# opentrack/neuralnet-tracker-traincode

Measured on AMD Instinct MI355X. Metric: face-crops/sec fwd+bwd @ batch 512, higher is better.
Workload: dtype f32; 1 GPU; NetworkWithPointHead(mobilenetv1, point head on, NLL off = training-script defaults): zero_grad + fwd + multi-task loss + bwd + fused clip/Adam step; per_gpu_batch=512, global_batch=512, input=129x129x1 f32, parallelism=dp1

## Files before the change

### neuralnet-tracker-traincode_amd/csrc/pw_bwd_fused.hip

```cpp
#include "ttk_common.h"
#include "conv_geom.h"

namespace ttk {

typedef float f32x16 __attribute__((ext_vector_type(16)));

constexpr int kFusedBM = 64;

template <int CIN, int COUT>
struct FusedShape {
  static constexpr int LDY = COUT + 4, LDC = CIN + 4, LDW = COUT + 4;
  static constexpr int NTC = CIN / 32, MTO = COUT / 32;
  static constexpr int DG = 2 * NTC;
  static constexpr int WG = MTO * NTC;
  static constexpr size_t smem_floats = (size_t)CIN * LDW + 2 * kFusedBM * LDY + 2 * kFusedBM * LDC + 4 * 2 * CIN;
};

template <int CIN, int COUT>
__global__ void __launch_bounds__(512) pw_bwd_fused_k(const float* __restrict__ g, const float* __restrict__ y, const float* __restrict__ bn_pw,
                                                       const float* __restrict__ w, const float* __restrict__ ydw,
                                                       const float* __restrict__ bn_dw, float* __restrict__ g_dw, float* __restrict__ dW,
                                                       float* __restrict__ wpartial, float* __restrict__ part, int64_t M, int ntiles) {
  using S = FusedShape<CIN, COUT>;
  constexpr int BM = kFusedBM, LDY = S::LDY, LDC = S::LDC, LDW = S::LDW, NTC = S::NTC, DG = S::DG, WG = S::WG;
  static_assert((CIN == 32 && COUT == 64) || (CIN == 64 && COUT == 128), "shapes of the first two pointwise layers");
  constexpr int DGW = DG >= 4 ? DG / 4 : 1, WGW = WG >= 4 ? WG / 4 : 1;
  static_assert(DGW == 1, "one data-gradient tile per consumer wave");
  __shared__ __attribute__((aligned(16))) float smem[S::smem_floats];
  float* Wt = smem;
  float* DyS = Wt + CIN * LDW;
  float* YcS = DyS + 2 * BM * LDY;
  float* red = YcS + 2 * BM * LDC;
  const int tid = threadIdx.x, lane = tid & 63, wave = tid >> 6;
  const bool producer = wave >= 4;
  const int r32 = lane & 31, h = lane >> 5;
  constexpr bool WG_PROD = false;
  const int wgw = WG_PROD ? wave - 4 : wave;
  const bool has_wg = WG_PROD ? producer : (!producer && (WG >= 4 || wave >= 4 - WG));
  const int wj0 = WG >= 4 ? wgw * WGW : wgw - (4 - WG);
  f32x16 wacc[WGW];
  float wsc[WGW], wbe[WGW];
#pragma unroll
  for (int j = 0; j < WGW; ++j) {
#pragma unroll
    for (int e = 0; e < 16; ++e) wacc[j][e] = 0.f;
    const int col = ((has_wg ? wj0 + j : 0) % NTC) * 32 + r32;
    wsc[j] = bn_dw[TTK_BN_SCALE * CIN + col];
    wbe[j] = bn_dw[TTK_BN_BETA * CIN + col];
  }
  auto wgrad_jobs = [&](int st, auto&& between) {
    const float* Dy = DyS + st * BM * LDY;
    const float* Yc = YcS + st * BM * LDC;
#pragma unroll
    for (int j = 0; j < WGW; ++j) {
      const int mt = (wj0 + j) / NTC, nt = (wj0 + j) % NTC;
      const float* ap = Dy + (4 * h) * LDY + mt * 32 + r32;
      const float* bp = Yc + (4 * h) * LDC + nt * 32 + r32;
      float a[2][4], b[2][4];
#pragma unroll
      for (int i = 0; i < 4; ++i) { a[0][i] = ap[i * LDY]; b[0][i] = bp[i * LDC]; }
#pragma unroll
      for (int q = 0; q < BM / 8; ++q) {
        const int cur = q & 1;
        if (q + 1 < BM / 8) {
#pragma unroll
          for (int i = 0; i < 4; ++i) { a[cur ^ 1][i] = ap[(8 * (q + 1) + i) * LDY]; b[cur ^ 1][i] = bp[(8 * (q + 1) + i) * LDC]; }
        }
        __builtin_amdgcn_sched_barrier(0);
#pragma unroll
        for (int i = 0; i < 4; ++i)
          wacc[j] = __builtin_amdgcn_mfma_f32_32x32x2f32(a[cur][i], fmaxf(fmaf(wsc[j], b[cur][i], wbe[j]), 0.f), wacc[j], 0, 0, 0);
        between(j * (BM / 8) + q);
        __builtin_amdgcn_sched_barrier(0);
      }
    }
  };

  for (int i = tid; i < CIN * COUT; i += 512) {
    const int co = i / CIN, ci = i - co * CIN;
    Wt[ci * LDW + co] = w[i];
  }

  if (producer) {
    const int pt = tid - 256;
    constexpr int QY = COUT / 4, QC = CIN / 4;
    constexpr int NY = BM * QY / 256, NC = BM * QC / 256;
    const int cy = pt % QY, cc = pt % QC;
    const float4 ga = ld4(bn_pw + TTK_BN_GA * COUT + 4 * cy), gb = ld4(bn_pw + TTK_BN_GB * COUT + 4 * cy);
    const float4 gmean = ld4(bn_pw + TTK_BN_GMEAN * COUT + 4 * cy), ymean = ld4(bn_pw + TTK_BN_MEAN * COUT + 4 * cy);
    const float4 dmean = ld4(bn_dw + TTK_BN_MEAN * CIN + 4 * cc);
    float4 rg[NY], ry[NY], rc[NC];
    auto load = [&](int t) {
      const int64_t m0 = (int64_t)t * BM;
#pragma unroll
      for (int i = 0; i < NY; ++i) {
        const int64_t row = m0 + (pt + 256 * i) / QY;
        const int64_t rcl = row < M ? row : M - 1;
        rg[i] = ld4nt(g + act_off(rcl, 4 * cy, M));
        ry[i] = ld4nt(y + act_off(rcl, 4 * cy, M));
      }
#pragma unroll
      for (int i = 0; i < NC; ++i) {
        const int64_t row = m0 + (pt + 256 * i) / QC;
        const int64_t rcl = row < M ? row : M - 1;
        rc[i] = ld4(ydw + act_off(rcl, 4 * cc, M));
      }
    };
    auto store = [&](int t, int st) {
      const int64_t m0 = (int64_t)t * BM;
#pragma unroll
      for (int i = 0; i < NY; ++i) {
        const int r = (pt + 256 * i) / QY;
        float4 v = fma4(ga, sub4(rg[i], gmean), mul4(gb, sub4(ry[i], ymean)));
        if (m0 + r >= M) v = f4(0.f);
        st4(DyS + (st * BM + r) * LDY + 4 * cy, v);
      }
#pragma unroll
      for (int i = 0; i < NC; ++i) {
        const int r = (pt + 256 * i) / QC;
        st4(YcS + (st * BM + r) * LDC + 4 * cc, sub4(rc[i], dmean));
      }
    };
    int t = blockIdx.x;
    if (t < ntiles) {
      load(t);
      store(t, 0);
      if (t + (int)gridDim.x < ntiles) load(t + gridDim.x);
    }
    __syncthreads();
    for (int it = 0; t < ntiles; t += gridDim.x, ++it) {
      const int tn = t + gridDim.x;
      if (tn < ntiles) {
        store(tn, (it + 1) & 1);
        if (tn + (int)gridDim.x < ntiles) load(tn + gridDim.x);
      }
      if constexpr (WG_PROD) wgrad_jobs(it & 1, [](int) {});
      __syncthreads();
    }
  } else {
    const bool has_dg = DG >= 4 || wave < DG;
    const int dj0 = DG >= 4 ? wave * DGW : wave;
    float s1[DGW], s2[DGW], dsc[DGW], dbe[DGW];
#pragma unroll
    for (int j = 0; j < DGW; ++j) {
      const int col = ((dj0 + j) % NTC) * 32 + r32;
      s1[j] = 0.f; s2[j] = 0.f;
      dsc[j] = has_dg ? bn_dw[TTK_BN_SCALE * CIN + col] : 0.f;
      dbe[j] = has_dg ? bn_dw[TTK_BN_BETA * CIN + col] : 0.f;
    }
    __syncthreads();
    int it = 0;
    for (int t = blockIdx.x; t < ntiles; t += gridDim.x, ++it) {
      const int st = it & 1;
      const float* Dy = DyS + st * BM * LDY;
      const float* Yc = YcS + st * BM * LDC;
      const int64_t m0 = (int64_t)t * BM;
      if (has_dg) {
#pragma unroll
        for (int j = 0; j < DGW; ++j) {
          const int mt = (dj0 + j) / NTC, nt = (dj0 + j) % NTC;
          f32x16 acc;
#pragma unroll
          for (int e = 0; e < 16; ++e) acc[e] = 0.f;
          const float* ap = Dy + (mt * 32 + r32) * LDY + 4 * h;
          const float* bp = Wt + (nt * 32 + r32) * LDW + 4 * h;
          float4 a4[2], b4[2];
          a4[0] = ld4(ap); b4[0] = ld4(bp);
#pragma unroll
          for (int q = 0; q < COUT / 8; ++q) {
            const int cur = q & 1;
            if (q + 1 < COUT / 8) { a4[cur ^ 1] = ld4(ap + 8 * (q + 1)); b4[cur ^ 1] = ld4(bp + 8 * (q + 1)); }
            __builtin_amdgcn_sched_barrier(0);
            acc = __builtin_amdgcn_mfma_f32_32x32x2f32(a4[cur].x, b4[cur].x, acc, 0, 0, 0);
            acc = __builtin_amdgcn_mfma_f32_32x32x2f32(a4[cur].y, b4[cur].y, acc, 0, 0, 0);
            acc = __builtin_amdgcn_mfma_f32_32x32x2f32(a4[cur].z, b4[cur].z, acc, 0, 0, 0);
            acc = __builtin_amdgcn_mfma_f32_32x32x2f32(a4[cur].w, b4[cur].w, acc, 0, 0, 0);
            __builtin_amdgcn_sched_barrier(0);
          }
          const int col = nt * 32 + r32;
          auto epi = [&](int e) {
            const int row = mt * 32 + (e & 3) + 8 * (e >> 2) + 4 * h;
            const float yc = Yc[row * LDC + col];
            const float out = fmaf(dsc[j], yc, dbe[j]) > 0.f ? acc[e] : 0.f;
            if (m0 + row < M) {
              g_dw[act_off(m0 + row, col, M)] = out;
              s1[j] += out;
              s2[j] = fmaf(out, yc, s2[j]);
            }
          };
          if constexpr (!WG_PROD && WG >= 4 && WGW * (BM / 8) == 16) {
            wgrad_jobs(st, epi);
          } else {
#pragma unroll
            for (int e = 0; e < 16; ++e) epi(e);
          }
        }
      }
      if constexpr (!WG_PROD && !(WG >= 4 && WGW * (BM / 8) == 16))
        if (has_wg) wgrad_jobs(st, [](int) {});
      __syncthreads();
    }
#pragma unroll
    for (int j = 0; j < DGW; ++j) {
      s1[j] += __shfl_xor(s1[j], 32);
      s2[j] += __shfl_xor(s2[j], 32);
    }
    if (has_dg && h == 0) {
      static_assert(DGW == 1, "one data-gradient tile per wave");
      red[(wave * 2 + 0) * CIN + (dj0 % NTC) * 32 + r32] = s1[0];
      red[(wave * 2 + 1) * CIN + (dj0 % NTC) * 32 + r32] = s2[0];
    }
  }
  if (has_wg) {
#pragma unroll
    for (int j = 0; j < WGW; ++j) {
      const int mt = (wj0 + j) / NTC, nt = (wj0 + j) % NTC;
#pragma unroll
      for (int e = 0; e < 16; ++e) {
        const int co = mt * 32 + (e & 3) + 8 * (e >> 2) + 4 * h, ci = nt * 32 + r32;
        if (wpartial) wpartial[(size_t)blockIdx.x * COUT * CIN + co * CIN + ci] = wacc[j][e];
        else atomicAdd(dW + co * CIN + ci, wacc[j][e]);
      }
    }
  }
  __syncthreads();
  if (part && tid < 2 * CIN) {
    const int which = tid / CIN, c = tid % CIN, nt = c / 32;
    float a = 0.f;
    for (int wv = 0; wv < (DG >= 4 ? 4 : DG); ++wv)
      if (wv % NTC == nt) a += red[(wv * 2 + which) * CIN + c];
    part[(size_t)blockIdx.x * 2 * CIN + which * CIN + c] = a;
  }
}


typedef _Float16 fz16x8 __attribute__((ext_vector_type(8)));
typedef _Float16 fz16x2 __attribute__((ext_vector_type(2)));
typedef float fz32x2 __attribute__((ext_vector_type(2)));
typedef float fz32x4 __attribute__((ext_vector_type(4)));

__device__ __forceinline__ int fz_swz(int row, int chunk) { return row * 32 + ((chunk ^ ((row >> 3) & 1)) << 4); }
__device__ __forceinline__ void fz_split(fz32x4 v, uint2& h, uint2& l) {
  const fz16x2 h01 = __builtin_convertvector(fz32x2{v.x, v.y}, fz16x2), h23 = __builtin_convertvector(fz32x2{v.z, v.w}, fz16x2);
  const fz32x2 f01 = __builtin_convertvector(h01, fz32x2), f23 = __builtin_convertvector(h23, fz32x2);
  const fz16x2 l01 = __builtin_convertvector(fz32x2{v.x - f01.x, v.y - f01.y}, fz16x2);
  const fz16x2 l23 = __builtin_convertvector(fz32x2{v.z - f23.x, v.w - f23.y}, fz16x2);
  h = make_uint2(__builtin_bit_cast(unsigned, h01), __builtin_bit_cast(unsigned, h23));
  l = make_uint2(__builtin_bit_cast(unsigned, l01), __builtin_bit_cast(unsigned, l23));
}

constexpr int kF16BM = 32;
template <int CIN, int COUT>
struct F16Shape {
  static constexpr int RowPlane = kF16BM * COUT * 2;
  static constexpr int TPlaneY = COUT * 32;
  static constexpr int TPlaneA = CIN * 32;
  static constexpr int Ldc = CIN + 4;
  static constexpr int Stage = 2 * RowPlane + 2 * 2 * TPlaneY + 2 * 2 * TPlaneA + kF16BM * Ldc * 4;
  static constexpr int NCI = CIN / 32, NCO = COUT / 32;
  static constexpr int GROUPS = 4 / NCI;
  static constexpr int COW = NCO / GROUPS;
};

template <int CIN, int COUT>
__global__ void __launch_bounds__(512) __attribute__((amdgpu_waves_per_eu(2, 2)))
pw_bwd_fused16_k(const float* __restrict__ g, const float* __restrict__ y, const float* __restrict__ bn_pw, const uint16_t* __restrict__ wq,
                 const float* __restrict__ wraw, const float* __restrict__ wmax, const float* __restrict__ ydw, const float* __restrict__ bn_dw, float* __restrict__ g_dw,
                 float* __restrict__ dW, float* __restrict__ wpartial, float* __restrict__ part, int64_t M, int ntiles) {
  using S_ = F16Shape<CIN, COUT>;
  constexpr int BM = kF16BM, NCI = S_::NCI, COW = S_::COW, kStage = S_::Stage, kRowPlane = S_::RowPlane, kTY = S_::TPlaneY, kTA = S_::TPlaneA,
                kLdc = S_::Ldc;
  static_assert((CIN == 128 || CIN == 64) && COUT == 128, "shapes");
  __shared__ __attribute__((aligned(16))) unsigned char lds[2 * kStage + 4 * 2 * 32 * 4];
  float* red = reinterpret_cast<float*>(lds + 2 * kStage);
  const int tid = threadIdx.x, lane = tid & 63, wave = tid >> 6;
  const bool producer = wave >= 4;
  const int r32 = lane & 31, h = lane >> 5;
  const float sa = pow2_scale(bn_pw[(size_t)TTK_BN_AUX * COUT + TTK_AUX_DY_BOUND]);
  const float sx = pow2_scale(bn_dw[(size_t)TTK_BN_AUX * CIN + TTK_AUX_ACT_BOUND]);
  const float sw = pow2_scale(*wmax);
  auto stage_ptr = [&](int st) { return lds + st * kStage; };

  if (producer) {
    const int pt = tid - 256;
    const int mb = pt & 7, cq = pt >> 3;
    const bool a_on = cq < CIN / 4;
    const int cqa = a_on ? cq : 0;
    const int sub = mb >> 2, chunk = (mb >> 1) & 1, o8 = (mb & 1) * 8;
    const fz32x4 ga = *reinterpret_cast<const fz32x4*>(bn_pw + TTK_BN_GA * COUT + 4 * cq) * sa;
    const fz32x4 gb = *reinterpret_cast<const fz32x4*>(bn_pw + TTK_BN_GB * COUT + 4 * cq) * sa;
    const fz32x4 gmean = *reinterpret_cast<const fz32x4*>(bn_pw + TTK_BN_GMEAN * COUT + 4 * cq);
    const fz32x4 ymean = *reinterpret_cast<const fz32x4*>(bn_pw + TTK_BN_MEAN * COUT + 4 * cq);
    const fz32x4 dsc = *reinterpret_cast<const fz32x4*>(bn_dw + TTK_BN_SCALE * CIN + 4 * cqa) * sx;
    const fz32x4 dbe = *reinterpret_cast<const fz32x4*>(bn_dw + TTK_BN_BETA * CIN + 4 * cqa) * sx;
    const fz32x4 dmean = *reinterpret_cast<const fz32x4*>(bn_dw + TTK_BN_MEAN * CIN + 4 * cqa);
    fz32x4 rg[4], ry[4], rc[4];
    auto load = [&](int t) {
      const int64_t r0 = (int64_t)t * BM + 4 * mb;
#pragma unroll
      for (int i = 0; i < 4; ++i) {
        const int64_t row = r0 + i < M ? r0 + i : M - 1;
        const float4 a = ld4nt(g + act_off(row, 4 * cq, M)), b = ld4nt(y + act_off(row, 4 * cq, M));
        rg[i] = fz32x4{a.x, a.y, a.z, a.w}; ry[i] = fz32x4{b.x, b.y, b.z, b.w};
        if (a_on) {
          const float4 c = ld4(ydw + act_off(row, 4 * cqa, M));
          rc[i] = fz32x4{c.x, c.y, c.z, c.w};
        }
      }
    };
    auto store = [&](int t, int st) {
      unsigned char* S = stage_ptr(st);
      unsigned char* DyR = S;
      unsigned char* DyT = S + 2 * kRowPlane;
      unsigned char* AT = DyT + 2 * 2 * kTY;
      float* Yc = reinterpret_cast<float*>(AT + 2 * 2 * kTA);
      const int64_t r0 = (int64_t)t * BM + 4 * mb;
      fz32x4 dy[4], av[4];
#pragma unroll
      for (int i = 0; i < 4; ++i) {
        dy[i] = ga * (rg[i] - gmean) + gb * (ry[i] - ymean);
        if (r0 + i >= M) dy[i] = fz32x4{0.f, 0.f, 0.f, 0.f};
        uint2 ph, pl;
        fz_split(dy[i], ph, pl);
        const int row = 4 * mb + i, off = row * (COUT * 2) + ((((cq >> 1) ^ (row & 15))) << 4) + (cq & 1) * 8;
        *reinterpret_cast<uint2*>(DyR + off) = ph;
        *reinterpret_cast<uint2*>(DyR + kRowPlane + off) = pl;
        if (a_on) {
          const fz32x4 yc = rc[i] - dmean;
          fz32x4 a = dsc * yc + dbe;
          a.x = fmaxf(a.x, 0.f); a.y = fmaxf(a.y, 0.f); a.z = fmaxf(a.z, 0.f); a.w = fmaxf(a.w, 0.f);
          if (r0 + i >= M) a = fz32x4{0.f, 0.f, 0.f, 0.f};
          av[i] = a;
          *reinterpret_cast<fz32x4*>(Yc + (4 * mb + i) * kLdc + 4 * cqa) = yc;
        }
      }
#pragma unroll
      for (int e = 0; e < 4; ++e) {
        uint2 ph, pl;
        fz_split(fz32x4{dy[0][e], dy[1][e], dy[2][e], dy[3][e]}, ph, pl);
        const int offy = sub * (2 * kTY) + fz_swz(4 * cq + e, chunk) + o8;
        *reinterpret_cast<uint2*>(DyT + offy) = ph;
        *reinterpret_cast<uint2*>(DyT + kTY + offy) = pl;
        if (a_on) {
          fz_split(fz32x4{av[0][e], av[1][e], av[2][e], av[3][e]}, ph, pl);
          const int offa = sub * (2 * kTA) + fz_swz(4 * cqa + e, chunk) + o8;
          *reinterpret_cast<uint2*>(AT + offa) = ph;
          *reinterpret_cast<uint2*>(AT + kTA + offa) = pl;
        }
      }
    };
    int t = blockIdx.x;
    if (t < ntiles) {
      load(t);
      store(t, 0);
      if (t + (int)gridDim.x < ntiles) load(t + gridDim.x);
    }
    __syncthreads();
    for (int it = 0; t < ntiles; t += gridDim.x, ++it) {
      const int tn = t + gridDim.x;
      if (tn < ntiles) {
        store(tn, (it + 1) & 1);
        if (tn + (int)gridDim.x < ntiles) load(tn + gridDim.x);
      }
      __syncthreads();
    }
  } else {
    const bool has_dg = wave < NCI;
    const int cit = wave % NCI, cog = wave / NCI;
    const int ci_dg = 32 * (has_dg ? wave : 0) + r32, ci_wg = 32 * cit + r32;
    fz16x8 Wf[COUT / 16][2];
#pragma unroll
    for (int s = 0; s < COUT / 16; ++s) {
      const int co = 16 * s + 8 * h;
      if (CIN == 128) {
        const size_t idx = ((size_t)(co >> 5) * CIN + ci_dg) * 32 + (co & 31);
        Wf[s][0] = *reinterpret_cast<const fz16x8*>(wq + idx);
        Wf[s][1] = *reinterpret_cast<const fz16x8*>(wq + (size_t)CIN * COUT + idx);
      } else {
#pragma unroll
        for (int e = 0; e < 8; ++e) {
          const float xs = wraw[(size_t)(co + e) * CIN + ci_dg] * sw;
          const _Float16 hh = (_Float16)xs;
          Wf[s][0][e] = hh;
          Wf[s][1][e] = (_Float16)(xs - (float)hh);
        }
      }
    }
    const float dsc = bn_dw[TTK_BN_SCALE * CIN + ci_dg], dbe = bn_dw[TTK_BN_BETA * CIN + ci_dg];
    const float inv_dg = 1.f / (sa * sw), inv_wg = 1.f / (sa * sx);
    f32x16 wacc[COW];
#pragma unroll
    for (int tt = 0; tt < COW; ++tt)
#pragma unroll
      for (int e = 0; e < 16; ++e) wacc[tt][e] = 0.f;
    float s1 = 0.f, s2 = 0.f;
    __syncthreads();
    int it = 0;
    for (int t = blockIdx.x; t < ntiles; t += gridDim.x, ++it) {
      const unsigned char* S = stage_ptr(it & 1);
      const unsigned char* DyR = S;
      const unsigned char* DyT = S + 2 * kRowPlane;
      const unsigned char* AT = DyT + 2 * 2 * kTY;
      const float* Yc = reinterpret_cast<const float*>(AT + 2 * 2 * kTA);
      const int64_t m0 = (int64_t)t * BM;
      f32x16 acc;
#pragma unroll
      for (int e = 0; e < 16; ++e) acc[e] = 0.f;
      if (has_dg) {
#pragma unroll
        for (int s = 0; s < COUT / 16; ++s) {
          const int off = r32 * (COUT * 2) + ((((2 * s + h) ^ (r32 & 15))) << 4);
          const fz16x8 ah = *reinterpret_cast<const fz16x8*>(DyR + off), al = *reinterpret_cast<const fz16x8*>(DyR + kRowPlane + off);
          acc = __builtin_amdgcn_mfma_f32_32x32x16_f16(ah, Wf[s][1], acc, 0, 0, 0);
          acc = __builtin_amdgcn_mfma_f32_32x32x16_f16(al, Wf[s][0], acc, 0, 0, 0);
          acc = __builtin_amdgcn_mfma_f32_32x32x16_f16(ah, Wf[s][0], acc, 0, 0, 0);
        }
      }
      fz16x8 bh[2], bl[2];
#pragma unroll
      for (int s = 0; s < 2; ++s) {
        const int off = s * (2 * kTA) + fz_swz(ci_wg, h);
        bh[s] = *reinterpret_cast<const fz16x8*>(AT + off);
        bl[s] = *reinterpret_cast<const fz16x8*>(AT + kTA + off);
      }
#pragma unroll
      for (int tt = 0; tt < COW; ++tt)
#pragma unroll
        for (int s = 0; s < 2; ++s) {
          const int off = s * (2 * kTY) + fz_swz(32 * (cog * COW + tt) + r32, h);
          const fz16x8 ah = *reinterpret_cast<const fz16x8*>(DyT + off), al = *reinterpret_cast<const fz16x8*>(DyT + kTY + off);
          wacc[tt] = __builtin_amdgcn_mfma_f32_32x32x16_f16(ah, bl[s], wacc[tt], 0, 0, 0);
          wacc[tt] = __builtin_amdgcn_mfma_f32_32x32x16_f16(al, bh[s], wacc[tt], 0, 0, 0);
          wacc[tt] = __builtin_amdgcn_mfma_f32_32x32x16_f16(ah, bh[s], wacc[tt], 0, 0, 0);
        }
      if (has_dg) {
#pragma unroll
        for (int e = 0; e < 16; ++e) {
          const int row = (e & 3) + 8 * (e >> 2) + 4 * h;
          const float yc = Yc[row * kLdc + ci_dg];
          const float out = fmaf(dsc, yc, dbe) > 0.f ? acc[e] * inv_dg : 0.f;
          if (m0 + row < M) {
            g_dw[act_off(m0 + row, ci_dg, M)] = out;
            s1 += out;
            s2 = fmaf(out, yc, s2);
          }
        }
      }
      __syncthreads();
    }
#pragma unroll
    for (int tt = 0; tt < COW; ++tt)
#pragma unroll
      for (int e = 0; e < 16; ++e) {
        const int co = 32 * (cog * COW + tt) + (e & 3) + 8 * (e >> 2) + 4 * h;
        const float v = wacc[tt][e] * inv_wg;
        if (wpartial) wpartial[(size_t)blockIdx.x * COUT * CIN + co * CIN + ci_wg] = v;
        else atomicAdd(dW + co * CIN + ci_wg, v);
      }
    s1 += __shfl_xor(s1, 32);
    s2 += __shfl_xor(s2, 32);
    if (h == 0 && has_dg) { red[(wave * 2 + 0) * 32 + r32] = s1; red[(wave * 2 + 1) * 32 + r32] = s2; }
  }
  __syncthreads();
  if (part && tid < 2 * CIN) {
    const int which = tid / CIN, c = tid % CIN;
    part[(size_t)blockIdx.x * 2 * CIN + which * CIN + c] = red[((c >> 5) * 2 + which) * 32 + (c & 31)];
  }
}

static bool fused_f16(int Cin) { return Cin == 128 || (Cin == 64 && gemm_mode() == GEMM_F16X2 && !exp_env("TTK_FUSED_FP32")); }
static bool fused_shape(int Cin, int Cout) {
  return (Cin == 32 && Cout == 64) || (Cin == 64 && Cout == 128) || (Cin == 128 && Cout == 128 && gemm_mode() == GEMM_F16X2);
}

static int fused_grid(int64_t M, int Cin) {
  const int64_t ntiles = ceil_div(M, fused_f16(Cin) ? kF16BM : kFusedBM);
  const int64_t cap = Cin == 32 ? 512 : 256;
  return (int)(ntiles < cap ? ntiles : cap);
}

}

using namespace ttk;

extern "C" {

int ttk_pwconv1x1_bwd_fused_rows(int64_t M, int Cin, int Cout) { return fused_shape(Cin, Cout) && M > 0 ? fused_grid(M, Cin) : 0; }

size_t ttk_pwconv1x1_bwd_fused_partial_bytes(int64_t M, int Cin, int Cout) {
  return fused_shape(Cin, Cout) && M > 0 ? (size_t)fused_grid(M, Cin) * Cin * Cout * sizeof(float) : 0;
}

int ttk_pwconv1x1_bwd_fused(const float* g, const float* y, const float* bn_pw, const float* w, const void* wsplit, const float* ydw,
                            const float* bn_dw, float* g_dw, float* dw, float* partial, float* part, int64_t M, int Cin, int Cout,
                            ttk_stream_t stream) {
  TTK_REQUIRE(g && y && bn_pw && ydw && bn_dw && g_dw && dw, "pwconv1x1_bwd_fused: null pointer");
  TTK_REQUIRE(fused_shape(Cin, Cout) && M > 0, "pwconv1x1_bwd_fused: only the 32 -> 64, 64 -> 128 and 128 -> 128 layers (got %d -> %d)", Cin, Cout);
  TTK_REQUIRE((Cin == 128 || w) && (!fused_f16(Cin) || wsplit),
              "pwconv1x1_bwd_fused: the fp16 forms (128 -> 128; 64 -> 128 in the default mode) need the prepared weight block, 32 -> 64 and 64 -> 128 the raw weights");
  const int ntiles = (int)ceil_div(M, fused_f16(Cin) ? kF16BM : kFusedBM), grid = fused_grid(M, Cin);
  hipStream_t st = (hipStream_t)stream;
  if (fused_f16(Cin)) {
    const size_t n = (size_t)Cin * Cout;
    const unsigned char* ws = static_cast<const unsigned char*>(wsplit);
    const uint16_t* wq = reinterpret_cast<const uint16_t*>(ws + prep_bwd_offset(n));
    const float* wmx = reinterpret_cast<const float*>(ws + prep_hdr_offset(n));
    if (Cin == 128)
      hipLaunchKernelGGL((pw_bwd_fused16_k<128, 128>), dim3(grid), dim3(512), 0, st, g, y, bn_pw, wq, w, wmx, ydw, bn_dw, g_dw, dw, partial, part, M, ntiles);
    else
      hipLaunchKernelGGL((pw_bwd_fused16_k<64, 128>), dim3(grid), dim3(512), 0, st, g, y, bn_pw, wq, w, wmx, ydw, bn_dw, g_dw, dw, partial, part, M, ntiles);
  } else if (Cin == 32) {
    hipLaunchKernelGGL((pw_bwd_fused_k<32, 64>), dim3(grid), dim3(512), 0, st, g, y, bn_pw, w, ydw, bn_dw, g_dw, dw, partial, part, M, ntiles);
  } else {
    hipLaunchKernelGGL((pw_bwd_fused_k<64, 128>), dim3(grid), dim3(512), 0, st, g, y, bn_pw, w, ydw, bn_dw, g_dw, dw, partial, part, M, ntiles);
  }
  if (partial) launch_fold_partials(partial, grid, (int64_t)Cin * Cout, dw, 1, st);
  TTK_LAUNCH_CHECK("pwconv1x1_bwd_fused");
}

}
```

Measured before the change: 69930 crops/s.

## Add fused fp16 pointwise backward kernel for 128->256 and 256->256 layers

Adds a new wide fused backward kernel for pointwise convs with 256 output channels. In one pass it computes the BN-folded dy, the input gradient through the depthwise BN/ReLU, the weight gradient and the BN partial sums, using split-fp16 MFMA and ds_read_tr transposed LDS reads. For 256 input channels the grid is split in two halves over input channels. The aim is to replace separate unfused kernels for these deeper layers and cut memory traffic and launches, at the cost of register pressure (waves_per_eu fixed at 2) and a row-count limit.

```diff
diff --git a/neuralnet-tracker-traincode_amd/csrc/pw_bwd_fused.hip b/neuralnet-tracker-traincode_amd/csrc/pw_bwd_fused.hip
--- a/neuralnet-tracker-traincode_amd/csrc/pw_bwd_fused.hip
+++ b/neuralnet-tracker-traincode_amd/csrc/pw_bwd_fused.hip
@@ -468,14 +468,248 @@
   }
 }
 
-static bool fused_f16(int Cin) { return Cin == 128 || (Cin == 64 && gemm_mode() == GEMM_F16X2 && !exp_env("TTK_FUSED_FP32")); }
+typedef short fzs16x4 __attribute__((ext_vector_type(4)));
+typedef short fzs16x8 __attribute__((ext_vector_type(8)));
+
+constexpr int kWideCW = 128;
+struct WideShape {
+  static constexpr int COUT = 256;
+  static constexpr int DyPlane = kF16BM * COUT * 2;
+  static constexpr int APlane = kWideCW * kF16BM * 2;
+  static constexpr int Ldc = kWideCW + 4;
+  static constexpr int Stage = 2 * DyPlane + 2 * APlane + kF16BM * Ldc * 4;
+};
+
+template <typename T> __device__ __forceinline__ T* wide_at(T* p, unsigned byte_off) {
+  return reinterpret_cast<T*>(reinterpret_cast<uintptr_t>(p) + byte_off);
+}
+__device__ __forceinline__ int wide_swz(int row) { return ((row & 3) << 2) | ((row >> 2) & 3); }
+
+__device__ __forceinline__ fz16x8 wide_tr_frag(const unsigned char* p0, const unsigned char* p1) {
+  const fzs16x4 lo = __builtin_amdgcn_ds_read_tr16_b64_v4i16((__attribute__((address_space(3))) fzs16x4*)(p0));
+  const fzs16x4 hi = __builtin_amdgcn_ds_read_tr16_b64_v4i16((__attribute__((address_space(3))) fzs16x4*)(p1));
+  const fzs16x8 v = __builtin_shufflevector(lo, hi, 0, 1, 2, 3, 4, 5, 6, 7);
+  return __builtin_bit_cast(fz16x8, v);
+}
+
+template <int CINT>
+__global__ void __launch_bounds__(512) __attribute__((amdgpu_waves_per_eu(2, 2)))
+pw_bwd_fused16w_k(const float* __restrict__ g, const float* __restrict__ y, const float* __restrict__ bn_pw, const float* __restrict__ wraw,
+                  const float* __restrict__ wmax, const float* __restrict__ ydw, const float* __restrict__ bn_dw, float* __restrict__ g_dw,
+                  float* __restrict__ dW, float* __restrict__ wpartial, float* __restrict__ part, int64_t M, int ntiles) {
+  using S_ = WideShape;
+  constexpr int BM = kF16BM, COUT = S_::COUT, CW = kWideCW, kStage = S_::Stage, kDyP = S_::DyPlane, kAP = S_::APlane, kLdc = S_::Ldc;
+  constexpr int HALVES = CINT / CW;
+  static_assert(CINT == 128 || CINT == 256, "shapes");
+  __shared__ __attribute__((aligned(16))) unsigned char lds[2 * kStage + (4 * COUT + 3 * CW + 2 * 512) * 4];
+  float* cpw = reinterpret_cast<float*>(lds + 2 * kStage);
+  float* cdw = cpw + 4 * COUT;
+  float* acc12 = cdw + 3 * CW;
+  const int tid = threadIdx.x, lane = tid & 63, wave = __builtin_amdgcn_readfirstlane(tid >> 6);
+  const int n16 = lane & 15, grp = lane >> 4;
+  auto fresh_tid = [&]() { int v = tid; asm volatile("" : "+v"(v)); return v; };
+  int walker = blockIdx.x, cio = 0, nwalk = gridDim.x;
+  if (HALVES == 2) {
+    nwalk = gridDim.x >> 1;
+    const int b = blockIdx.x, b0 = (nwalk & ~7) * 2;
+    walker = b < b0 ? (b >> 4) * 8 + (b & 7) : (nwalk & ~7) + ((b - b0) >> 1);
+    cio = (b < b0 ? (b >> 3) & 1 : (b - b0) & 1) * CW;
+  }
+  auto uni = [](float v) { return __builtin_bit_cast(float, __builtin_amdgcn_readfirstlane(__builtin_bit_cast(int, v))); };
+  const float sa = uni(pow2_scale(bn_pw[(size_t)TTK_BN_AUX * COUT + TTK_AUX_DY_BOUND]));
+  const float sx = uni(pow2_scale(bn_dw[(size_t)TTK_BN_AUX * CINT + TTK_AUX_ACT_BOUND]));
+  const float sw = uni(pow2_scale(*wmax));
+
+  for (int i = tid; i < COUT; i += 512) {
+    cpw[i] = bn_pw[TTK_BN_GA * COUT + i] * sa;
+    cpw[COUT + i] = bn_pw[TTK_BN_GB * COUT + i] * sa;
+    cpw[2 * COUT + i] = bn_pw[TTK_BN_GMEAN * COUT + i];
+    cpw[3 * COUT + i] = bn_pw[TTK_BN_MEAN * COUT + i];
+  }
+  for (int i = tid; i < CW; i += 512) {
+    cdw[i] = bn_dw[TTK_BN_SCALE * CINT + cio + i] * sx;
+    cdw[CW + i] = bn_dw[TTK_BN_BETA * CINT + cio + i] * sx;
+    cdw[2 * CW + i] = bn_dw[TTK_BN_MEAN * CINT + cio + i];
+  }
+  __syncthreads();
+
+  const unsigned Mu = (unsigned)M;
+  fz32x4 rg[4], ry[4], rc[2];
+  auto load = [&](int t) {
+    const int ft = fresh_tid(), mb = ft & 7, cq = ft >> 3, rp = (wave & 1) * 8 + ((ft & 63) >> 3), cqa = (wave >> 1) * 8 + (ft & 7);
+    const unsigned r0 = (unsigned)t * BM + 4 * mb, q0 = (unsigned)t * BM + 2 * rp;
+#pragma unroll
+    for (int i = 0; i < 4; ++i) {
+      const unsigned row = r0 + i < Mu ? r0 + i : Mu - 1;
+      const unsigned off = (((cq >> 3) * Mu + row) * kCB + 4 * (cq & 7)) * 4;
+      const float4 a = ld4nt(wide_at(g, off)), b = ld4nt(wide_at(y, off));
+      rg[i] = fz32x4{a.x, a.y, a.z, a.w}; ry[i] = fz32x4{b.x, b.y, b.z, b.w};
+    }
+#pragma unroll
+    for (int i = 0; i < 2; ++i) {
+      const unsigned row = q0 + i < Mu ? q0 + i : Mu - 1;
+      const float4 c = ld4(wide_at(ydw, ((((cio >> 5) + (cqa >> 3)) * Mu + row) * kCB + 4 * (cqa & 7)) * 4));
+      rc[i] = fz32x4{c.x, c.y, c.z, c.w};
+    }
+  };
+  auto store = [&](int t, int st) {
+    const int ft = fresh_tid(), mb = ft & 7, cq = ft >> 3, rp = (wave & 1) * 8 + ((ft & 63) >> 3), cqa = (wave >> 1) * 8 + (ft & 7);
+    const int dyoff = (cq >> 5) * (kDyP / 2) + 4 * mb * 256 + (((((cq & 31) >> 1) ^ (mb & 3))) << 4) + (cq & 1) * 8;
+    unsigned char* S = lds + st * kStage;
+    unsigned char* DyR = S;
+    unsigned char* AT = S + 2 * kDyP;
+    float* Yc = reinterpret_cast<float*>(AT + 2 * kAP);
+    const unsigned r0 = (unsigned)t * BM + 4 * mb, q0 = (unsigned)t * BM + 2 * rp;
+    {
+      const fz32x4 dsc = *reinterpret_cast<const fz32x4*>(cdw + 4 * cqa), dbe = *reinterpret_cast<const fz32x4*>(cdw + CW + 4 * cqa);
+      const fz32x4 dmean = *reinterpret_cast<const fz32x4*>(cdw + 2 * CW + 4 * cqa);
+      fz32x4 av[2];
+#pragma unroll
+      for (int i = 0; i < 2; ++i) {
+        const fz32x4 yc = rc[i] - dmean;
+        fz32x4 a = dsc * yc + dbe;
+        a.x = fmaxf(a.x, 0.f); a.y = fmaxf(a.y, 0.f); a.z = fmaxf(a.z, 0.f); a.w = fmaxf(a.w, 0.f);
+        if (q0 + i >= Mu) a = fz32x4{0.f, 0.f, 0.f, 0.f};
+        av[i] = a;
+        *reinterpret_cast<fz32x4*>(Yc + (2 * rp + i) * kLdc + 4 * cqa) = yc;
+      }
+#pragma unroll
+      for (int e = 0; e < 4; ++e) {
+        const fz32x2 v{av[0][e], av[1][e]};
+        const fz16x2 vh = __builtin_convertvector(v, fz16x2);
+        const fz16x2 vl = __builtin_convertvector(v - __builtin_convertvector(vh, fz32x2), fz16x2);
+        const int offa = (4 * cqa + e) * 64 + ((((rp >> 2) ^ (cqa & 3))) << 4) + (rp & 3) * 4;
+        *reinterpret_cast<unsigned*>(AT + offa) = __builtin_bit_cast(unsigned, vh);
+        *reinterpret_cast<unsigned*>(AT + kAP + offa) = __builtin_bit_cast(unsigned, vl);
+      }
+    }
+    __builtin_amdgcn_sched_barrier(0);
+    const fz32x4 ga = *reinterpret_cast<const fz32x4*>(cpw + 4 * cq), gb = *reinterpret_cast<const fz32x4*>(cpw + COUT + 4 * cq);
+    const fz32x4 gmean = *reinterpret_cast<const fz32x4*>(cpw + 2 * COUT + 4 * cq), ymean = *reinterpret_cast<const fz32x4*>(cpw + 3 * COUT + 4 * cq);
+#pragma unroll
+    for (int i = 0; i < 4; ++i) {
+      fz32x4 dy = ga * (rg[i] - gmean) + gb * (ry[i] - ymean);
+      if (r0 + i >= Mu) dy = fz32x4{0.f, 0.f, 0.f, 0.f};
+      uint2 ph, pl;
+      fz_split(dy, ph, pl);
+      const int off = (dyoff ^ (i << 6)) + i * 256;
+      *reinterpret_cast<uint2*>(DyR + off) = ph;
+      *reinterpret_cast<uint2*>(DyR + kDyP + off) = pl;
+      __builtin_amdgcn_sched_barrier(0);
+    }
+  };
+
+  const int cil = 16 * wave + n16, ci = cio + cil;
+  fz16x8 Wf[COUT / 32][2];
+#pragma unroll
+  for (int s = 0; s < COUT / 32; ++s)
+#pragma unroll
+    for (int e = 0; e < 8; ++e) {
+      const float xs = wraw[(size_t)(32 * s + 8 * grp + e) * CINT + ci] * sw;
+      const _Float16 hh = (_Float16)xs;
+      Wf[s][0][e] = hh;
+      Wf[s][1][e] = (_Float16)(xs - (float)hh);
+    }
+  const float inv_dg = uni(1.f / (sa * sw)), inv_wg = uni(1.f / (sa * sx));
+  fz32x4 wacc[COUT / 16];
+#pragma unroll
+  for (int ct = 0; ct < COUT / 16; ++ct) wacc[ct] = fz32x4{0.f, 0.f, 0.f, 0.f};
+  acc12[tid] = 0.f; acc12[512 + tid] = 0.f;
+  auto compute = [&](int st, int t) {
+    const int ft = fresh_tid(), n16 = ft & 15, grp = (ft & 63) >> 4, cil = 16 * wave + n16, ci = cio + cil;
+    const int rbase = n16 * 256 + ((grp ^ wide_swz(n16)) << 4);
+    const int tq = n16 >> 2, tp = n16 & 3;
+    const int tb0 = (8 * grp + tq) * 256 + ((((tp >> 1) ^ wide_swz(8 * grp + tq))) << 4) + (tp & 1) * 8;
+    const int aoff = cil * 64 + ((grp ^ ((cil >> 2) & 3)) << 4);
+    const unsigned char* S = lds + st * kStage;
+    const unsigned char* DyR = S;
+    const unsigned char* AT = S + 2 * kDyP;
+    const float* Yc = reinterpret_cast<const float*>(AT + 2 * kAP);
+    const unsigned m0 = (unsigned)t * BM;
+    fz32x4 acc[2] = {fz32x4{0.f, 0.f, 0.f, 0.f}, fz32x4{0.f, 0.f, 0.f, 0.f}};
+#pragma unroll
+    for (int s = 0; s < COUT / 32; ++s)
+#pragma unroll
+      for (int rt = 0; rt < 2; ++rt) {
+        const int off = (rbase ^ (64 * (s & 3))) + (s >> 2) * (kDyP / 2) + rt * 16 * 256;
+        const fz16x8 ah = *reinterpret_cast<const fz16x8*>(DyR + off), al = *reinterpret_cast<const fz16x8*>(DyR + kDyP + off);
+        acc[rt] = __builtin_amdgcn_mfma_f32_16x16x32_f16(ah, Wf[s][1], acc[rt], 0, 0, 0);
+        acc[rt] = __builtin_amdgcn_mfma_f32_16x16x32_f16(al, Wf[s][0], acc[rt], 0, 0, 0);
+        acc[rt] = __builtin_amdgcn_mfma_f32_16x16x32_f16(ah, Wf[s][0], acc[rt], 0, 0, 0);
+      }
+    const fz16x8 bh = *reinterpret_cast<const fz16x8*>(AT + aoff), bl = *reinterpret_cast<const fz16x8*>(AT + kAP + aoff);
+#pragma unroll
+    for (int ct = 0; ct < COUT / 16; ++ct) {
+      const int o0 = (tb0 ^ (32 * (ct & 7))) + (ct >> 3) * (kDyP / 2), o1 = (tb0 ^ (32 * (ct & 7) ^ 16)) + (ct >> 3) * (kDyP / 2) + 4 * 256;
+      const fz16x8 ah = wide_tr_frag(DyR + o0, DyR + o1), al = wide_tr_frag(DyR + kDyP + o0, DyR + kDyP + o1);
+      wacc[ct] = __builtin_amdgcn_mfma_f32_16x16x32_f16(ah, bl, wacc[ct], 0, 0, 0);
+      wacc[ct] = __builtin_amdgcn_mfma_f32_16x16x32_f16(al, bh, wacc[ct], 0, 0, 0);
+      wacc[ct] = __builtin_amdgcn_mfma_f32_16x16x32_f16(ah, bh, wacc[ct], 0, 0, 0);
+    }
+    const float dsc1 = cdw[cil], dbe1 = cdw[CW + cil];
+    float s1 = acc12[tid], s2 = acc12[512 + tid];
+#pragma unroll
+    for (int rt = 0; rt < 2; ++rt)
+#pragma unroll
+      for (int r = 0; r < 4; ++r) {
+        const int row = 16 * rt + 4 * grp + r;
+        const float yc = Yc[row * kLdc + cil];
+        const float out = fmaf(dsc1, yc, dbe1) > 0.f ? acc[rt][r] * inv_dg : 0.f;
+        if (m0 + row < Mu) {
+          *wide_at(g_dw, (((ci >> 5) * Mu + m0 + row) * kCB + (ci & 31)) * 4) = out;
+          s1 += out;
+          s2 = fmaf(out, yc, s2);
+        }
+      }
+    acc12[tid] = s1; acc12[512 + tid] = s2;
+  };
+
+  int t = walker;
+  if (t < ntiles) {
+    load(t);
+    store(t, 0);
+    if (t + nwalk < ntiles) load(t + nwalk);
+  }
+  __syncthreads();
+  for (int it = 0; t < ntiles; t += nwalk, ++it) {
+    const int tn = t + nwalk;
+    if (tn < ntiles) {
+      store(tn, (it + 1) & 1);
+      if (tn + nwalk < ntiles) load(tn + nwalk);
+    }
+    compute(it & 1, t);
+    __syncthreads();
+  }
+#pragma unroll
+  for (int ct = 0; ct < COUT / 16; ++ct)
+#pragma unroll
+    for (int r = 0; r < 4; ++r) {
+      const int co = 16 * ct + 4 * grp + r;
+      const float v = wacc[ct][r] * inv_wg;
+      if (wpartial) wpartial[(size_t)walker * COUT * CINT + co * CINT + ci] = v;
+      else atomicAdd(dW + co * CINT + ci, v);
+    }
+  if (part && tid < 2 * CW) {
+    const int which = tid / CW, c = tid % CW;
+    const float* src = acc12 + which * 512 + 64 * (c >> 4) + (c & 15);
+    part[(size_t)walker * 2 * CINT + which * CINT + cio + c] = (src[0] + src[16]) + (src[32] + src[48]);
+  }
+}
+
+static bool fused_f16(int Cin) { return Cin == 128 || Cin == 256 || (Cin == 64 && gemm_mode() == GEMM_F16X2 && !exp_env("TTK_FUSED_FP32")); }
+static bool fused_wide(int Cin, int Cout) {
+  static const int only = [] { const char* e = exp_env("TTK_FUSED_WIDE"); return e ? atoi(e) : -1; }();
+  return Cout == 256 && (Cin == 128 || Cin == 256) && (only < 0 || only == Cin);
+}
+constexpr int64_t kWideMaxM = ((int64_t)1 << 30) / 256 - kF16BM;
 static bool fused_shape(int Cin, int Cout) {
-  return (Cin == 32 && Cout == 64) || (Cin == 64 && Cout == 128) || (Cin == 128 && Cout == 128 && gemm_mode() == GEMM_F16X2);
-}
-
-static int fused_grid(int64_t M, int Cin) {
+  return (Cin == 32 && Cout == 64) || (Cin == 64 && Cout == 128) ||
+         (((Cin == 128 && Cout == 128) || fused_wide(Cin, Cout)) && gemm_mode() == GEMM_F16X2);
+}
+
+static int fused_grid(int64_t M, int Cin, int Cout) {
   const int64_t ntiles = ceil_div(M, fused_f16(Cin) ? kF16BM : kFusedBM);
-  const int64_t cap = Cin == 32 ? 512 : 256;
+  const int64_t cap = Cin == 32 ? 512 : (fused_wide(Cin, Cout) && Cin == 256 ? 128 : 256);
   return (int)(ntiles < cap ? ntiles : cap);
 }
 
@@ -485,27 +719,33 @@
 
 extern "C" {
 
-int ttk_pwconv1x1_bwd_fused_rows(int64_t M, int Cin, int Cout) { return fused_shape(Cin, Cout) && M > 0 ? fused_grid(M, Cin) : 0; }
+static bool fused_ok(int64_t M, int Cin, int Cout) { return fused_shape(Cin, Cout) && M > 0 && !(fused_wide(Cin, Cout) && M > kWideMaxM); }
+
+int ttk_pwconv1x1_bwd_fused_rows(int64_t M, int Cin, int Cout) { return fused_ok(M, Cin, Cout) ? fused_grid(M, Cin, Cout) : 0; }
 
 size_t ttk_pwconv1x1_bwd_fused_partial_bytes(int64_t M, int Cin, int Cout) {
-  return fused_shape(Cin, Cout) && M > 0 ? (size_t)fused_grid(M, Cin) * Cin * Cout * sizeof(float) : 0;
+  return fused_ok(M, Cin, Cout) ? (size_t)fused_grid(M, Cin, Cout) * Cin * Cout * sizeof(float) : 0;
 }
 
 int ttk_pwconv1x1_bwd_fused(const float* g, const float* y, const float* bn_pw, const float* w, const void* wsplit, const float* ydw,
                             const float* bn_dw, float* g_dw, float* dw, float* partial, float* part, int64_t M, int Cin, int Cout,
                             ttk_stream_t stream) {
   TTK_REQUIRE(g && y && bn_pw && ydw && bn_dw && g_dw && dw, "pwconv1x1_bwd_fused: null pointer");
-  TTK_REQUIRE(fused_shape(Cin, Cout) && M > 0, "pwconv1x1_bwd_fused: only the 32 -> 64, 64 -> 128 and 128 -> 128 layers (got %d -> %d)", Cin, Cout);
-  TTK_REQUIRE((Cin == 128 || w) && (!fused_f16(Cin) || wsplit),
-              "pwconv1x1_bwd_fused: the fp16 forms (128 -> 128; 64 -> 128 in the default mode) need the prepared weight block, 32 -> 64 and 64 -> 128 the raw weights");
-  const int ntiles = (int)ceil_div(M, fused_f16(Cin) ? kF16BM : kFusedBM), grid = fused_grid(M, Cin);
+  TTK_REQUIRE(fused_ok(M, Cin, Cout), "pwconv1x1_bwd_fused: only the 32 -> 64, 64 -> 128, 128 -> 128, 128 -> 256 and 256 -> 256 layers (got %d -> %d)", Cin, Cout);
+  TTK_REQUIRE(((Cin == 128 && Cout == 128) || w) && (!fused_f16(Cin) || wsplit),
+              "pwconv1x1_bwd_fused: the fp16 forms (128 and more input channels; 64 -> 128 in the default mode) need the prepared weight block, all but 128 -> 128 the raw weights");
+  const int ntiles = (int)ceil_div(M, fused_f16(Cin) ? kF16BM : kFusedBM), grid = fused_grid(M, Cin, Cout);
   hipStream_t st = (hipStream_t)stream;
   if (fused_f16(Cin)) {
     const size_t n = (size_t)Cin * Cout;
     const unsigned char* ws = static_cast<const unsigned char*>(wsplit);
     const uint16_t* wq = reinterpret_cast<const uint16_t*>(ws + prep_bwd_offset(n));
     const float* wmx = reinterpret_cast<const float*>(ws + prep_hdr_offset(n));
-    if (Cin == 128)
+    if (fused_wide(Cin, Cout) && Cin == 128)
+      hipLaunchKernelGGL((pw_bwd_fused16w_k<128>), dim3(grid), dim3(512), 0, st, g, y, bn_pw, w, wmx, ydw, bn_dw, g_dw, dw, partial, part, M, ntiles);
+    else if (fused_wide(Cin, Cout))
+      hipLaunchKernelGGL((pw_bwd_fused16w_k<256>), dim3(2 * grid), dim3(512), 0, st, g, y, bn_pw, w, wmx, ydw, bn_dw, g_dw, dw, partial, part, M, ntiles);
+    else if (Cin == 128)
       hipLaunchKernelGGL((pw_bwd_fused16_k<128, 128>), dim3(grid), dim3(512), 0, st, g, y, bn_pw, wq, w, wmx, ydw, bn_dw, g_dw, dw, partial, part, M, ntiles);
     else
       hipLaunchKernelGGL((pw_bwd_fused16_k<64, 128>), dim3(grid), dim3(512), 0, st, g, y, bn_pw, wq, w, wmx, ydw, bn_dw, g_dw, dw, partial, part, M, ntiles);
```

After: 71220 crops/s (median of 6 runs). 1.8% higher.
